# jbikker/tinybvh

Measured on NVIDIA B200. Metric: Mrays/s (primary+shadow), higher is better.
Workload: dtype f32

## Files before the change

### tinybvh_b200/csrc/common.cuh

```cuda
#pragma once
#include <cuda_runtime.h>
#include <stdint.h>
#include <stdio.h>
#include <mutex>
#include <vector>
#include <atomic>
#include "../../include/tinybvh_b200.h"

#define BVH_FAR 1e30f
#define TBVH_STACK 64
#define TBVH_STACK_DEEP 256

void tbvh_set_error( const char* fmt, ... );
extern unsigned long long g_tbvh_launches;
#define CUDA_TRY( x ) do { cudaError_t e_ = (x); if (e_ != cudaSuccess) { tbvh_set_error( "%s:%d %s -> %s", __FILE__, __LINE__, #x, cudaGetErrorString( e_ ) ); return TBVH_E_CUDA; } } while (0)
#define LAUNCHED() do { g_tbvh_launches++; cudaError_t e_ = cudaGetLastError(); if (e_ != cudaSuccess) { tbvh_set_error( "%s:%d launch -> %s", __FILE__, __LINE__, cudaGetErrorString( e_ ) ); return TBVH_E_CUDA; } } while (0)

struct HostSlot
{
	void* d_rays = 0;
	void* d_hits = 0;
	void* d_bits = 0;
	void* h_hits = 0;
	cudaEvent_t in_done = 0, run_done = 0, out_done = 0;
};
#define TBVH_SLOTS 4

struct tbvh_ctx_t
{
	int device = 0;
	int sm_count = 148;
	int numa_node = -1;
	cudaStream_t stream = 0;
	std::mutex host_mutex;
	cudaStream_t s_in = 0, s_run = 0, s_out = 0;
	cudaStream_t s_in_part[3] = { 0, 0, 0 };
	cudaEvent_t ev_part[TBVH_SLOTS][3] = {};
	cudaEvent_t ev_fork = 0;
	HostSlot slot[TBVH_SLOTS];
	size_t chunk_rays = 1u << 19;
	size_t slot_rays = 0;
	size_t slot_rec = 0;
	int host_path = 0;
	int h2d_split = 1;
	int d2h_mode = 1;
	int scatter_threads = 8;
	struct HostPool* pool = 0;
	int trace_variant = 3;
	int small_mode = 0;
	int inst_idx_bits = 32;
	int hq_small = 16;
	int hq_cluster = 16;
	int small_t = 128;
	int build_ctas = 0;
	int build_mode = 0;
	unsigned long long* d_counters = 0;
	std::atomic<uint32_t> counter_next{ 0 };
};
#define TBVH_COUNTERS 256

uint32_t tbvh_next_generation();
struct BlasLink { tbvh_bvh blas; uint32_t generation; };

struct tbvh_bvh_t
{
	tbvh_ctx ctx = 0;
	tbvh_info info = {};
	float4* d_verts = 0;
	float4* d_nodes = 0;
	uint32_t* d_prim_idx = 0;
	float4* d_trav = 0;
	uint32_t root_ref = 0, root_count = 0;
	float4* d_leaf_tris = 0;
	uint32_t leaf_tris_count = 0;
	float4* d_nodes_gpu = 0;
	float4* d_cw_nodes = 0;
	float4* d_cw_tris = 0;
	float4* d_cw_trav = 0;
	uint32_t cw_depth = 0;
	uint32_t generation = 0;
	float4* d_aabbs = 0;
	void* d_inst = 0;
	void* d_blas = 0;
	uint32_t inst_count = 0, blas_count = 0;
	uint32_t tlas_blas_layouts = 0;
	std::vector<BlasLink> links;
	bool refittable = true;
	int stats = 0;
	unsigned long long* d_stats = 0;
};


__device__ __forceinline__ bool mt_test( const float ox, const float oy, const float oz, const float dx, const float dy, const float dz,
	const float4 v0, const float4 e1, const float4 e2, const float tmax, float& t, float& u, float& v )
{
	const float hx = __fmaf_rn( dy, e2.z, -__fmul_rn( dz, e2.y ) );
	const float hy = __fmaf_rn( dz, e2.x, -__fmul_rn( dx, e2.z ) );
	const float hz = __fmaf_rn( dx, e2.y, -__fmul_rn( dy, e2.x ) );
	const float a = __fmaf_rn( e1.z, hz, __fmaf_rn( e1.x, hx, __fmul_rn( e1.y, hy ) ) );
	if (fabsf( a ) < 0.000001f) return false;
	const float f = __fdiv_rn( 1.0f, a );
	const float sx = __fsub_rn( ox, v0.x ), sy = __fsub_rn( oy, v0.y ), sz = __fsub_rn( oz, v0.z );
	u = __fmul_rn( f, __fmaf_rn( hz, sz, __fmaf_rn( hx, sx, __fmul_rn( hy, sy ) ) ) );
	const float qx = __fmaf_rn( -e1.y, sz, __fmul_rn( e1.z, sy ) );
	const float qy = __fmaf_rn( -e1.z, sx, __fmul_rn( e1.x, sz ) );
	const float qz = __fmaf_rn( -e1.x, sy, __fmul_rn( e1.y, sx ) );
	v = __fmul_rn( f, __fmaf_rn( dz, qz, __fmaf_rn( dy, qy, __fmul_rn( dx, qx ) ) ) );
	if (u < 0 || v < 0 || __fadd_rn( u, v ) > 1) return false;
	t = __fmul_rn( f, __fmaf_rn( e2.z, qz, __fmaf_rn( e2.x, qx, __fmul_rn( e2.y, qy ) ) ) );
	return !(t < 0 || t > tmax);
}

__device__ __forceinline__ uint32_t f2key( float f ) { uint32_t u = __float_as_uint( f ); return (u & 0x80000000u) ? ~u : (u | 0x80000000u); }
__device__ __forceinline__ float key2f( uint32_t k ) { return __uint_as_float( (k & 0x80000000u) ? (k & 0x7fffffffu) : ~k ); }

int bvh2_trace_launch( tbvh_bvh b, const void* d_rays, uint32_t stride, void* d_hits, uint32_t hit_stride, uint32_t* d_bits, uint64_t n, bool anyhit, cudaStream_t s, unsigned long long* d_stats );
int cwbvh_trace_launch( tbvh_bvh b, const void* d_rays, uint32_t stride, void* d_hits, uint32_t hit_stride, uint32_t* d_bits, uint64_t n, bool anyhit, cudaStream_t s, unsigned long long* d_stats );
int cw_make_trav( tbvh_bvh b, cudaStream_t s, int known_depth = -1 );
unsigned long long* ctx_next_counter( tbvh_ctx c );
int build_sah_launch( tbvh_bvh b, float c_trav, float c_int, int flavour );
int build_hq_launch( tbvh_bvh b, float c_trav, float c_int );
int refit_launch( tbvh_bvh b, cudaStream_t s );
int tlas_trace_launch( tbvh_bvh b, int layout, const void* d_rays, uint32_t stride, uint32_t* d_bits, uint64_t n, bool anyhit, cudaStream_t s );
struct TlasInst { float inv[16]; uint32_t blasIdx, mask, pad0, pad1; };
struct BlasRef { const float4* trav; const float4* tris; uint32_t root_ref, root_count, pad0, pad1; const float4* cw_nodes; const float4* cw_tris; };
int make_leaf_tris( tbvh_bvh b, cudaStream_t s );
int bvh_gpu_to_bvh( tbvh_bvh b, uint32_t used_nodes_gpu, cudaStream_t s );
int bvh_to_bvh_gpu( tbvh_bvh b, cudaStream_t s );
int bvh_to_cwbvh( tbvh_bvh b, cudaStream_t s );
int exclusive_scan( const uint32_t* in, uint32_t* out, uint32_t* tile_sum, uint32_t n, cudaStream_t s );
```

### tinybvh_b200/csrc/cw_walk.cuh

```cuda
#pragma once
#include "common.cuh"
#include <cuda_fp16.h>

#define CW_STACK 128
#define CW_NODE_F4 10
#ifndef CW_PLANES_BF16
#define CW_PLANES_BF16 0
#endif

__device__ __forceinline__ float2 widen( const uint32_t h2 )
{
#if CW_PLANES_BF16
	return make_float2( __uint_as_float( h2 * 65536u ), __uint_as_float( h2 & 0xffff0000u ) );
#else
	return __half22float2( *(const __half2*)&h2 );
#endif
}

__device__ __forceinline__ uint32_t pair_hits( const uint32_t wnx, const uint32_t wny, const uint32_t wnz, const uint32_t wfx, const uint32_t wfy, const uint32_t wfz,
	const uint32_t bits_a, const uint32_t bits_b, const float2 ax, const float2 ay, const float2 az, const float2 bx, const float2 by, const float2 bz, const float t )
{
	const float2 tnx = __ffma2_rn( widen( wnx ), ax, bx ), tny = __ffma2_rn( widen( wny ), ay, by ), tnz = __ffma2_rn( widen( wnz ), az, bz );
	const float2 tfx = __ffma2_rn( widen( wfx ), ax, bx ), tfy = __ffma2_rn( widen( wfy ), ay, by ), tfz = __ffma2_rn( widen( wfz ), az, bz );
	const float in_a = fmaxf( fmaxf( fmaxf( tnx.x, tny.x ), tnz.x ), 0.0f ), out_a = fminf( fminf( fminf( tfx.x, tfy.x ), tfz.x ), t );
	const float in_b = fmaxf( fmaxf( fmaxf( tnx.y, tny.y ), tnz.y ), 0.0f ), out_b = fminf( fminf( fminf( tfx.y, tfy.y ), tfz.y ), t );
	return (in_a <= out_a ? bits_a : 0u) | (in_b <= out_b ? bits_b : 0u);
}

__device__ __forceinline__ uint32_t slots_to_order( const uint32_t w, const uint32_t o )
{
	uint32_t top = w >> 24;
	if (o & 1u) top = ((top & 0x55u) << 1) | ((top >> 1) & 0x55u);
	if (o & 2u) top = ((top & 0x33u) << 2) | ((top >> 2) & 0x33u);
	if (o & 4u) top = ((top & 0x0fu) << 4) | (top >> 4);
	return top << 24;
}

template <int OCT> __device__ __forceinline__ uint32_t node_hits( const float4* __restrict__ np, const uint32_t pairs, const bool negx, const bool negy, const bool negz, const uint32_t o,
	const float ax1, const float ay1, const float az1, const float bx1, const float by1, const float bz1, const float t )
{
	const bool nx = OCT < 0 ? negx : (OCT & 4) != 0, ny = OCT < 0 ? negy : (OCT & 2) != 0, nz = OCT < 0 ? negz : (OCT & 1) != 0;
	const float2 ax = make_float2( ax1, ax1 ), ay = make_float2( ay1, ay1 ), az = make_float2( az1, az1 );
	const float2 bx = make_float2( bx1, bx1 ), by = make_float2( by1, by1 ), bz = make_float2( bz1, bz1 );
	(void)pairs;
	float4 A[4], B[4];
	#pragma unroll
	for (int j = 0; j < 4; j++) A[j] = __ldg( np + 2 + 2 * j ), B[j] = __ldg( np + 3 + 2 * j );
	uint32_t got = 0;
	#pragma unroll
	for (int j = 0; j < 4; j++)
	{
		const uint32_t lx = __float_as_uint( A[j].x ), ly = __float_as_uint( A[j].y ), lz = __float_as_uint( A[j].z );
		const uint32_t hx = __float_as_uint( A[j].w ), hy = __float_as_uint( B[j].x ), hz = __float_as_uint( B[j].y );
		got |= pair_hits( nx ? hx : lx, ny ? hy : ly, nz ? hz : lz, nx ? lx : hx, ny ? ly : hy, nz ? lz : hz,
			__float_as_uint( B[j].z ), __float_as_uint( B[j].w ), ax, ay, az, bx, by, bz, t );
	}
	return slots_to_order( got, OCT < 0 ? o : (uint32_t)(7 - OCT) ) | (got & 0x00ffffffu);
}
```

### tinybvh_b200/csrc/multi.cu

```cuda
#include "common.cuh"
#include <sched.h>
#include <sys/mman.h>
#include <string.h>
#include <thread>
#include <string>
#include <vector>
#include <new>

struct tbvh_group_t
{
	std::vector<tbvh_ctx> ctx;
	std::vector<tbvh_bvh> replica;
	std::vector<char> owned;
	std::vector<std::pair<void*, size_t>> host_blocks;
};

#define ARG_CHECK( c, msg ) do { if (!(c)) { tbvh_set_error( "%s: %s", __func__, msg ); return TBVH_E_ARG; } } while (0)
#define TRY( x ) do { int r_ = (x); if (r_ != TBVH_OK) return r_; } while (0)

static void release_replicas( tbvh_group g )
{
	for (size_t i = 0; i < g->replica.size(); i++) if (g->replica[i] && g->owned[i]) tbvh_bvh_destroy( g->replica[i] );
	g->replica.clear(), g->owned.clear();
}

static int peer_clone( void** dst, int dst_dev, const void* src, int src_dev, size_t bytes, cudaStream_t s )
{
	*dst = 0;
	if (!src || bytes == 0) return TBVH_OK;
	CUDA_TRY( cudaMalloc( dst, bytes ) );
	CUDA_TRY( cudaMemcpyPeerAsync( *dst, dst_dev, src, src_dev, bytes, s ) );
	return TBVH_OK;
}

template <class F> static int per_device( tbvh_group g, F fn )
{
	const size_t parts = g->ctx.size();
	std::vector<int> rc( parts, TBVH_OK );
	std::vector<std::string> msg( parts );
	std::vector<std::thread> th;
	for (size_t p = 0; p < parts; p++) th.emplace_back( [&, p]()
	{
		tbvh_bind_thread_to_device( g->ctx[p]->device );
		rc[p] = fn( (uint32_t)p );
		if (rc[p] != TBVH_OK) msg[p] = tbvh_last_error();
	} );
	for (auto& t : th) t.join();
	for (size_t p = 0; p < parts; p++) if (rc[p] != TBVH_OK) { tbvh_set_error( "device %d: %s", g->ctx[p]->device, msg[p].c_str() ); return rc[p]; }
	return TBVH_OK;
}

extern "C" {

void tbvh_shard_range( uint64_t n, uint32_t part, uint32_t parts, uint64_t* first, uint64_t* count )
{
	const uint64_t units = (n + 31) / 32;
	const uint64_t lo = units * part / parts, hi = units * (part + 1) / parts;
	const uint64_t a = lo * 32 < n ? lo * 32 : n, e = hi * 32 < n ? hi * 32 : n;
	if (first) *first = a;
	if (count) *count = e - a;
}

int tbvh_group_create( const int* devices, int count, tbvh_group* out )
{
	ARG_CHECK( out, "out == NULL" );
	int have = 0;
	CUDA_TRY( cudaGetDeviceCount( &have ) );
	if (count <= 0) count = have, devices = 0;
	ARG_CHECK( count >= 1 && count <= 64, "device count out of range" );
	for (int i = 0; i < count; i++) ARG_CHECK( (devices ? devices[i] : i) >= 0 && (devices ? devices[i] : i) < have, "no such device" );
	tbvh_group g = new (std::nothrow) tbvh_group_t();
	ARG_CHECK( g, "out of host memory" );
	for (int i = 0; i < count; i++)
	{
		const int dev = devices ? devices[i] : i;
		tbvh_ctx c = 0;
		const int rc = tbvh_ctx_create( dev, &c );
		if (rc != TBVH_OK) { for (tbvh_ctx x : g->ctx) tbvh_ctx_destroy( x ); delete g; return rc; }
		g->ctx.push_back( c );
	}
	for (int i = 0; i < count; i++) for (int j = 0; j < count; j++) if (i != j)
	{
		int can = 0;
		cudaDeviceCanAccessPeer( &can, g->ctx[i]->device, g->ctx[j]->device );
		if (can) { cudaSetDevice( g->ctx[i]->device ); if (cudaDeviceEnablePeerAccess( g->ctx[j]->device, 0 ) != cudaSuccess) cudaGetLastError(); }
	}
	*out = g;
	return TBVH_OK;
}

int tbvh_group_destroy( tbvh_group g )
{
	if (!g) return TBVH_OK;
	release_replicas( g );
	for (auto& b : g->host_blocks) { cudaHostUnregister( b.first ); munmap( b.first, b.second ); }
	for (tbvh_ctx c : g->ctx) tbvh_ctx_destroy( c );
	delete g;
	return TBVH_OK;
}

int tbvh_group_size( tbvh_group g ) { return g ? (int)g->ctx.size() : 0; }
tbvh_ctx tbvh_group_ctx( tbvh_group g, int i ) { return g && i >= 0 && i < (int)g->ctx.size() ? g->ctx[i] : 0; }
tbvh_bvh tbvh_group_replica( tbvh_group g, int i ) { return g && i >= 0 && i < (int)g->replica.size() ? g->replica[i] : 0; }

int tbvh_group_replicate( tbvh_group g, tbvh_bvh src, double* ms_out )
{
	ARG_CHECK( g && src, "NULL argument" );
	if (src->d_inst) { tbvh_set_error( "tbvh_group_replicate: a TLAS points into its BLAS handles and cannot be replicated by itself" ); return TBVH_E_UNSUPPORTED; }
	if (!(src->info.layouts & (1u << TBVH_LAYOUT_BVH)) && !src->d_cw_trav) { tbvh_set_error( "tbvh_group_replicate: the source holds no tree" ); return TBVH_E_STATE; }
	release_replicas( g );
	const int sdev = src->ctx->device;
	CUDA_TRY( cudaSetDevice( sdev ) );
	CUDA_TRY( cudaStreamSynchronize( src->ctx->stream ) );
	cudaEvent_t e0 = 0, e1 = 0;
	CUDA_TRY( cudaEventCreate( &e0 ) );
	CUDA_TRY( cudaEventCreate( &e1 ) );
	CUDA_TRY( cudaEventRecord( e0, src->ctx->stream ) );
	int rc = TBVH_OK;
	for (size_t i = 0; i < g->ctx.size() && rc == TBVH_OK; i++)
	{
		tbvh_ctx c = g->ctx[i];
		if (c == src->ctx) { g->replica.push_back( src ), g->owned.push_back( 0 ); continue; }
		tbvh_bvh r = 0;
		rc = tbvh_bvh_create( c, &r );
		if (rc != TBVH_OK) break;
		g->replica.push_back( r ), g->owned.push_back( 1 );
		auto body = [&]() -> int
		{
			CUDA_TRY( cudaSetDevice( c->device ) );
			cudaStream_t s = c->stream;
			r->info = src->info, r->root_ref = src->root_ref, r->root_count = src->root_count, r->refittable = src->refittable, r->cw_depth = src->cw_depth;
			const size_t nodes_b = (size_t)(src->info.used_nodes < 2 ? 2 : src->info.used_nodes) * 32;
			TRY( peer_clone( (void**)&r->d_verts, c->device, src->d_verts, sdev, (size_t)src->info.prim_count * 48, s ) );
			TRY( peer_clone( (void**)&r->d_prim_idx, c->device, src->d_prim_idx, sdev, (size_t)src->info.idx_count * 4, s ) );
			if (src->d_nodes) TRY( peer_clone( (void**)&r->d_nodes, c->device, src->d_nodes, sdev, nodes_b, s ) );
			if (src->d_trav == src->d_nodes) r->d_trav = r->d_nodes;
			else if (src->d_trav) TRY( peer_clone( (void**)&r->d_trav, c->device, src->d_trav, sdev, (size_t)src->info.used_nodes_gpu * 64, s ) );
			if (src->d_leaf_tris) { TRY( peer_clone( (void**)&r->d_leaf_tris, c->device, src->d_leaf_tris, sdev, (size_t)src->leaf_tris_count * 48, s ) ); r->leaf_tris_count = src->leaf_tris_count; }
			if (src->d_nodes_gpu) TRY( peer_clone( (void**)&r->d_nodes_gpu, c->device, src->d_nodes_gpu, sdev, (size_t)src->info.used_nodes_gpu * 64, s ) );
			if (src->d_cw_nodes) TRY( peer_clone( (void**)&r->d_cw_nodes, c->device, src->d_cw_nodes, sdev, (size_t)src->info.used_blocks * 16, s ) );
			if (src->d_cw_tris) TRY( peer_clone( (void**)&r->d_cw_tris, c->device, src->d_cw_tris, sdev, (size_t)src->info.cwbvh_tri_count * 48, s ) );
			if (src->d_cw_trav) TRY( peer_clone( (void**)&r->d_cw_trav, c->device, src->d_cw_trav, sdev, (size_t)(src->info.used_blocks / 5) * 160, s ) );
			return TBVH_OK;
		};
		rc = body();
	}
	for (tbvh_ctx c : g->ctx) { cudaSetDevice( c->device ); cudaStreamSynchronize( c->stream ); }
	cudaSetDevice( sdev );
	cudaEventRecord( e1, src->ctx->stream );
	cudaEventSynchronize( e1 );
	float ms = 0;
	cudaEventElapsedTime( &ms, e0, e1 );
	if (ms_out) *ms_out = ms;
	cudaEventDestroy( e0 ), cudaEventDestroy( e1 );
	if (rc != TBVH_OK) release_replicas( g );
	return rc;
}

int tbvh_group_intersect( tbvh_group g, int layout, void* rays, uint32_t stride, uint64_t n )
{
	ARG_CHECK( g && rays && stride >= 64, "bad arguments" );
	if (g->replica.size() != g->ctx.size()) { tbvh_set_error( "tbvh_group_intersect: call tbvh_group_replicate first" ); return TBVH_E_STATE; }
	const uint32_t parts = (uint32_t)g->ctx.size();
	return per_device( g, [&]( uint32_t p ) -> int
	{
		uint64_t first, count;
		tbvh_shard_range( n, p, parts, &first, &count );
		if (count == 0) return TBVH_OK;
		return tbvh_intersect( g->replica[p], layout, (char*)rays + first * stride, stride, count );
	} );
}

int tbvh_group_occluded( tbvh_group g, int layout, const void* rays, uint32_t stride, uint64_t n, uint32_t* bits )
{
	ARG_CHECK( g && rays && bits && stride >= 64, "bad arguments" );
	if (g->replica.size() != g->ctx.size()) { tbvh_set_error( "tbvh_group_occluded: call tbvh_group_replicate first" ); return TBVH_E_STATE; }
	const uint32_t parts = (uint32_t)g->ctx.size();
	return per_device( g, [&]( uint32_t p ) -> int
	{
		uint64_t first, count;
		tbvh_shard_range( n, p, parts, &first, &count );
		if (count == 0) return TBVH_OK;
		return tbvh_occluded( g->replica[p], layout, (const char*)rays + first * stride, stride, count, bits + first / 32 );
	} );
}

int tbvh_group_host_alloc( tbvh_group g, uint32_t stride, uint64_t n, void** out )
{
	ARG_CHECK( g && out && stride > 0 && n > 0, "bad arguments" );
	const size_t bytes = ((size_t)stride * n + 4095) & ~(size_t)4095;
	void* p = mmap( 0, bytes, PROT_READ | PROT_WRITE, MAP_PRIVATE | MAP_ANONYMOUS, -1, 0 );
	if (p == MAP_FAILED) { tbvh_set_error( "tbvh_group_host_alloc: mmap( %zu ) failed", bytes ); return TBVH_E_ARG; }
	const uint32_t parts = (uint32_t)g->ctx.size();
	per_device( g, [&]( uint32_t part ) -> int
	{
		uint64_t first, count;
		tbvh_shard_range( n, part, parts, &first, &count );
		char* a = (char*)p + first * stride, * e = a + count * stride;
		if (part + 1 == parts) e = (char*)p + bytes;
		for (char* q = (char*)((uintptr_t)a & ~(uintptr_t)4095); q < e; q += 4096) *(volatile char*)q = 0;
		return TBVH_OK;
	} );
	const cudaError_t err = cudaHostRegister( p, bytes, cudaHostRegisterPortable );
	if (err != cudaSuccess) { munmap( p, bytes ); tbvh_set_error( "tbvh_group_host_alloc: cudaHostRegister -> %s", cudaGetErrorString( err ) ); return TBVH_E_CUDA; }
	g->host_blocks.push_back( { p, bytes } );
	*out = p;
	return TBVH_OK;
}

int tbvh_group_host_free( tbvh_group g, void* p )
{
	ARG_CHECK( g, "NULL group" );
	for (size_t i = 0; i < g->host_blocks.size(); i++) if (g->host_blocks[i].first == p)
	{
		cudaHostUnregister( p );
		munmap( p, g->host_blocks[i].second );
		g->host_blocks.erase( g->host_blocks.begin() + i );
		return TBVH_OK;
	}
	tbvh_set_error( "tbvh_group_host_free: not a block of this group" );
	return TBVH_E_ARG;
}

}
```

### tinybvh_b200/csrc/trace_cwbvh.cu

```cuda
#include "cw_walk.cuh"
#include <vector>

__global__ void k_cw_expand( const uint4* __restrict__ src, uint4* __restrict__ dst, uint32_t* __restrict__ parent, const uint32_t count )
{
	const uint32_t x = blockIdx.x * blockDim.x + threadIdx.x;
	if (x >= count) return;
	const uint4 n0 = src[(size_t)x * 5], n1 = src[(size_t)x * 5 + 1], n2 = src[(size_t)x * 5 + 2], n3 = src[(size_t)x * 5 + 3], n4 = src[(size_t)x * 5 + 4];
	const uint32_t row[6][2] = { { n2.x, n2.y }, { n2.z, n2.w }, { n3.x, n3.y }, { n3.z, n3.w }, { n4.x, n4.y }, { n4.z, n4.w } };
	const uint32_t meta[2] = { n1.z, n1.w };
	uint32_t word[4][8];
	#pragma unroll
	for (int j = 0; j < 4; j++) for (int k = 0; k < 8; k++) word[j][k] = 0;
	uint32_t kept = 0, inner = 0;
	#pragma unroll
	for (int i = 0; i < 8; i++)
	{
		const uint32_t m = (meta[i >> 2] >> (8 * (i & 3))) & 255u;
		if (m == 0) continue;
		const bool is_inner = (m & 0x18u) == 0x18u;
		const uint32_t bits = is_inner ? 1u << (24u + (m & 7u)) : (m >> 5) << (m & 31u);
		if (is_inner) inner++;
		const uint32_t j = kept >> 1, side = kept & 1;
		#pragma unroll
		for (int r = 0; r < 6; r++)
		{
			const uint32_t q = (row[r][i >> 2] >> (8 * (i & 3))) & 255u;
			const uint32_t h = CW_PLANES_BF16 ? __float_as_uint( (float)q ) >> 16 : (uint32_t)__half_as_ushort( __uint2half_rn( q ) );
			#pragma unroll
			for (int jj = 0; jj < 4; jj++) if (jj == (int)j) word[jj][r] |= side ? h << 16 : h;
		}
		#pragma unroll
		for (int jj = 0; jj < 4; jj++) if (jj == (int)j) word[jj][6 + side] = bits;
		kept++;
	}
	uint4* o = dst + (size_t)x * CW_NODE_F4;
	const uint32_t sx = (uint32_t)(((int)(int8_t)(n0.w & 255u) + 127) * 128) & 0xffffu, sy = (uint32_t)(((int)(int8_t)((n0.w >> 8) & 255u) + 127) * 128) & 0xffffu;
	const uint32_t sz = (uint32_t)(((int)(int8_t)((n0.w >> 16) & 255u) + 127) * 128) & 0xffffu;
	o[0] = make_uint4( n0.x, n0.y, n0.z, sx | (sy << 16) );
	o[1] = make_uint4( n1.x, n1.y, sz | ((n0.w >> 24) << 16) | (((kept + 1) >> 1) << 24), kept );
	#pragma unroll
	for (int j = 0; j < 4; j++)
	{
		o[2 + 2 * j] = make_uint4( word[j][0], word[j][1], word[j][2], word[j][3] );
		o[3 + 2 * j] = make_uint4( word[j][4], word[j][5], word[j][6], word[j][7] );
	}
	if (parent) for (uint32_t c = 0; c < inner; c++) if (n1.x + c < count) parent[n1.x + c] = x;
}

__global__ void k_cw_depth( const uint32_t* __restrict__ parent, const uint32_t count, uint32_t* __restrict__ max_depth )
{
	const uint32_t x = blockIdx.x * blockDim.x + threadIdx.x;
	if (x >= count) return;
	uint32_t d = 0, n = x;
	while (n != 0 && n < count && d < 4096) n = parent[n], d++;
	if (n != 0) return;
	atomicMax( max_depth, d );
}

int cw_make_trav( tbvh_bvh b, cudaStream_t s, int known_depth )
{
	if (b->d_cw_trav) cudaFree( b->d_cw_trav ), b->d_cw_trav = 0;
	const uint32_t count = b->info.used_blocks / 5;
	if (count == 0) { tbvh_set_error( "cw_make_trav: no CWBVH nodes" ); return TBVH_E_STATE; }
	CUDA_TRY( cudaMalloc( &b->d_cw_trav, (size_t)count * CW_NODE_F4 * 16 ) );
	if (known_depth >= 0)
	{
		k_cw_expand<<<(count + 127) / 128, 128, 0, s>>>( (const uint4*)b->d_cw_nodes, (uint4*)b->d_cw_trav, 0, count ); LAUNCHED();
		b->cw_depth = (uint32_t)known_depth;
		return TBVH_OK;
	}
	uint32_t* d_parent = 0;
	CUDA_TRY( cudaMalloc( &d_parent, ((size_t)count + 1) * 4 ) );
	uint32_t depth = 0;
	auto body = [&]() -> int
	{
		CUDA_TRY( cudaMemsetAsync( d_parent, 0xff, (size_t)count * 4, s ) );
		CUDA_TRY( cudaMemsetAsync( d_parent + count, 0, 4, s ) );
		k_cw_expand<<<(count + 127) / 128, 128, 0, s>>>( (const uint4*)b->d_cw_nodes, (uint4*)b->d_cw_trav, d_parent, count ); LAUNCHED();
		k_cw_depth<<<(count + 127) / 128, 128, 0, s>>>( d_parent, count, d_parent + count ); LAUNCHED();
		CUDA_TRY( cudaMemcpyAsync( &depth, d_parent + count, 4, cudaMemcpyDeviceToHost, s ) );
		CUDA_TRY( cudaStreamSynchronize( s ) );
		return TBVH_OK;
	};
	const int rc = body();
	cudaFree( d_parent );
	b->cw_depth = depth;
	return rc;
}


template <bool ANYHIT, bool STATS, int OCTSW>
__global__ void __launch_bounds__( 128 ) k_trace_wide( const float4* __restrict__ nodes, const float4* __restrict__ tris,
	const char* rays, const uint32_t stride, char* hits, const uint32_t hit_stride, uint32_t* __restrict__ bits, const uint64_t n,
	unsigned long long* __restrict__ stats )
{
	const uint64_t i = (uint64_t)blockIdx.x * blockDim.x + threadIdx.x;
	bool occluded = false;
	const bool valid = i < n;
	float4 ro4 = make_float4( 0, 0, 0, 0 ), rd4 = ro4, rr4 = ro4, rh4 = ro4;
	if (valid)
	{
		const float4* rp = (const float4*)(rays + i * stride);
		ro4 = rp[0], rd4 = rp[1], rr4 = rp[2], rh4 = rp[3];
	}
	const float ox = ro4.x, oy = ro4.y, oz = ro4.z, dx = rd4.x, dy = rd4.y, dz = rd4.z;
	const float rdx = rr4.x, rdy = rr4.y, rdz = rr4.z;
	const uint32_t o = 7u - ((dx < 0 ? 4u : 0u) | (dy < 0 ? 2u : 0u) | (dz < 0 ? 1u : 0u));
	const bool negx = rdx < 0, negy = rdy < 0, negz = rdz < 0;
	const uint32_t oct = (negx ? 4u : 0u) | (negy ? 2u : 0u) | (negz ? 1u : 0u);
	bool uni = false;
	if (OCTSW)
	{
		const uint32_t vm = __ballot_sync( 0xffffffffu, valid );
		const uint32_t oct0 = __shfl_sync( 0xffffffffu, oct, vm ? __ffs( vm ) - 1 : 0 );
		uni = __all_sync( 0xffffffffu, !valid || (oct == oct0 && o == 7u - oct) );
	}
	if (valid)
	{
		float t = rh4.x, hu = rh4.y, hv = rh4.z;
		uint32_t hprim = __float_as_uint( rh4.w );
		uint2 pending[CW_STACK];
		int depth = 0;
		uint32_t base = 0, word = 0x80000000u;
		unsigned long long nsteps = 0, ntris = 0, npairs = 0;
		while (true)
		{
			const uint32_t bit = 31u - __clz( word );
			const uint32_t rest = word & ~(1u << bit);
			if (rest > 0x00ffffffu) pending[depth++] = make_uint2( base, rest );
			const uint32_t slot = (bit - 24u) ^ o;
			const uint32_t nidx = base + __popc( word & ~(0xffffffffu << slot) );
			const float4* np = nodes + (size_t)nidx * CW_NODE_F4;
			const float4 h0 = __ldg( np ), h1 = __ldg( np + 1 );
			if (STATS) nsteps++;
			const uint32_t sxy = __float_as_uint( h0.w ), szm = __float_as_uint( h1.z );
			const float scx = __uint_as_float( sxy << 16 ), scy = __uint_as_float( sxy & 0xffff0000u ), scz = __uint_as_float( szm << 16 );
			const float ax1 = __fmul_rn( scx, rdx ), ay1 = __fmul_rn( scy, rdy ), az1 = __fmul_rn( scz, rdz );
			const float bx1 = __fmul_rn( -__fsub_rn( ox, h0.x ), rdx ), by1 = __fmul_rn( -__fsub_rn( oy, h0.y ), rdy ), bz1 = __fmul_rn( -__fsub_rn( oz, h0.z ), rdz );
			const uint32_t pairs = szm >> 24;
			if (STATS) npairs += pairs;
			uint32_t got;
			#define NODE_HITS( O ) got = node_hits<O>( np, pairs, negx, negy, negz, o, ax1, ay1, az1, bx1, by1, bz1, t )
			if (OCTSW && uni)
			{
				switch (oct)
				{
				case 0: NODE_HITS( 0 ); break;
				case 1: NODE_HITS( 1 ); break;
				case 2: NODE_HITS( 2 ); break;
				case 3: NODE_HITS( 3 ); break;
				case 4: NODE_HITS( 4 ); break;
				case 5: NODE_HITS( 5 ); break;
				case 6: NODE_HITS( 6 ); break;
				default: NODE_HITS( 7 ); break;
				}
			}
			else NODE_HITS( -1 );
			#undef NODE_HITS
			base = __float_as_uint( h1.x );
			word = (got & 0xff000000u) | ((szm >> 16) & 255u);
			uint32_t tmask = got & 0x00ffffffu;
			const float4* tbase = tris + __float_as_uint( h1.y );
			while (tmask)
			{
				const uint32_t k = 31u - __clz( tmask );
				tmask &= ~(1u << k);
				const float4* tp = tbase + k * 3;
				const float4 e2 = __ldg( tp ), e1 = __ldg( tp + 1 ), v0 = __ldg( tp + 2 );
				if (STATS) ntris++;
				float tt, u, v;
				if (mt_test( ox, oy, oz, dx, dy, dz, v0, e1, e2, t, tt, u, v ))
				{
					if (ANYHIT) { occluded = true; break; }
					t = tt, hu = u, hv = v, hprim = __float_as_uint( v0.w );
				}
			}
			if (ANYHIT && occluded) break;
			if (word > 0x00ffffffu) continue;
			if (depth == 0) break;
			const uint2 e = pending[--depth];
			base = e.x, word = e.y;
		}
		if (!ANYHIT)
		{
			float4* hp = (float4*)(hits + i * hit_stride);
			*hp = make_float4( t, hu, hv, __uint_as_float( hprim ) );
		}
		if (STATS) { atomicAdd( &stats[0], nsteps ); atomicAdd( &stats[1], ntris ); atomicAdd( &stats[2], npairs ); }
	}
	if (ANYHIT)
	{
		const uint32_t m = __ballot_sync( 0xffffffffu, occluded );
		if ((threadIdx.x & 31) == 0 && (i & ~31ull) < n) bits[i >> 5] = m;
	}
}

int cwbvh_trace_launch( tbvh_bvh b, const void* d_rays, uint32_t stride, void* d_hits, uint32_t hit_stride, uint32_t* d_bits,
	uint64_t n, bool anyhit, cudaStream_t s, unsigned long long* d_stats )
{
	if (!b->d_cw_trav || !b->d_cw_tris) { tbvh_set_error( "CWBVH layout not resident" ); return TBVH_E_STATE; }
	if (n == 0) return TBVH_OK;
	if (b->cw_depth + 1 > CW_STACK) { tbvh_set_error( "wide-tree depth %u exceeds the %d pending node groups a ray can hold (the reference's own limit)", b->cw_depth, CW_STACK ); return TBVH_E_LIMIT; }
	const uint32_t block = 128;
	const uint64_t grid = (n + block - 1) / block;
	if (grid > 0x7fffffffull) { tbvh_set_error( "ray batch too large for one launch" ); return TBVH_E_ARG; }
	const int sw = b->ctx->trace_variant == 0 ? 0 : 1;
	#define LAUNCH( A, S, O ) k_trace_wide<A, S, O><<<(uint32_t)grid, block, 0, s>>>( b->d_cw_trav, b->d_cw_tris, (const char*)d_rays, stride, \
		(char*)d_hits, hit_stride, d_bits, n, d_stats )
	if (anyhit) { if (d_stats) LAUNCH( true, true, 0 ); else if (sw) LAUNCH( true, false, 1 ); else LAUNCH( true, false, 0 ); }
	else { if (d_stats) LAUNCH( false, true, 0 ); else if (sw) LAUNCH( false, false, 1 ); else LAUNCH( false, false, 0 ); }
	#undef LAUNCH
	LAUNCHED();
	return TBVH_OK;
}
```

### tinybvh_b200/csrc/trace_tlas.cu

```cuda
#include "cw_walk.cuh"

#define TLAS_STACK 64

namespace
{
__device__ __forceinline__ float safercp( const float x ) { return (x > 1e-12f || x < -1e-12f) ? __fdiv_rn( 1.0f, x ) : (x >= 0 ? BVH_FAR : -BVH_FAR); }

__device__ __forceinline__ bool slab( const float4 c0, const float4 c1, const bool px, const bool py, const bool pz, const float rdx, const float rdy, const float rdz,
	const float nrox, const float nroy, const float nroz, const float tmax, float& tmin )
{
	const float tx1 = __fmaf_rn( px ? c0.x : c1.x, rdx, nrox ), tx2 = __fmaf_rn( px ? c1.x : c0.x, rdx, nrox );
	const float ty1 = __fmaf_rn( py ? c0.y : c1.y, rdy, nroy ), ty2 = __fmaf_rn( py ? c1.y : c0.y, rdy, nroy );
	const float tz1 = __fmaf_rn( pz ? c0.z : c1.z, rdz, nroz ), tz2 = __fmaf_rn( pz ? c1.z : c0.z, rdz, nroz );
	tmin = fmaxf( fmaxf( tx1, ty1 ), fmaxf( tz1, 0.0f ) );
	return fminf( fminf( tx2, ty2 ), fminf( tz2, tmax ) ) >= tmin;
}

template <bool ANYHIT> __device__ bool trace_blas( const BlasRef B, const float ox, const float oy, const float oz, const float dx, const float dy, const float dz,
	const float rdx, const float rdy, const float rdz, float& tmax, float& hu, float& hv, uint32_t& hprim, bool& hit, uint2* stack )
{
	const bool px = dx >= 0, py = dy >= 0, pz = dz >= 0;
	const float nrox = -__fmul_rn( ox, rdx ), nroy = -__fmul_rn( oy, rdy ), nroz = -__fmul_rn( oz, rdz );
	int sp = 0;
	uint32_t ref = B.root_ref, cnt = B.root_count;
	while (true)
	{
		if (cnt == 0)
		{
			const float4* p = B.trav + (size_t)ref * 2;
			const float4 a0 = __ldg( p ), a1 = __ldg( p + 1 ), b0 = __ldg( p + 2 ), b1 = __ldg( p + 3 );
			float tmina, tminb;
			const bool hita = slab( a0, a1, px, py, pz, rdx, rdy, rdz, nrox, nroy, nroz, tmax, tmina );
			const bool hitb = slab( b0, b1, px, py, pz, rdx, rdy, rdz, nrox, nroy, nroz, tmax, tminb );
			const uint32_t refa = __float_as_uint( a0.w ), cnta = __float_as_uint( a1.w ), refb = __float_as_uint( b0.w ), cntb = __float_as_uint( b1.w );
			if (hita && hitb)
			{
				const bool swp = tmina > tminb;
				ref = swp ? refb : refa, cnt = swp ? cntb : cnta;
				stack[sp++] = swp ? make_uint2( refa, cnta ) : make_uint2( refb, cntb );
				continue;
			}
			if (hita) { ref = refa, cnt = cnta; continue; }
			if (hitb) { ref = refb, cnt = cntb; continue; }
		}
		else
		{
			const float4* tp = B.tris + (size_t)ref * 3;
			for (uint32_t k = 0; k < cnt; k++, tp += 3)
			{
				const float4 v0 = __ldg( tp ), e1 = __ldg( tp + 1 ), e2 = __ldg( tp + 2 );
				float t, u, v;
				if (mt_test( ox, oy, oz, dx, dy, dz, v0, e1, e2, tmax, t, u, v ))
				{
					if (ANYHIT) return true;
					tmax = t, hu = u, hv = v, hprim = __float_as_uint( v0.w ), hit = true;
				}
			}
		}
		if (sp == 0) break;
		const uint2 e = stack[--sp];
		ref = e.x, cnt = e.y;
	}
	return false;
}

template <bool ANYHIT> __device__ bool trace_blas_cw( const float4* __restrict__ nodes, const float4* __restrict__ tris, const float ox, const float oy, const float oz,
	const float dx, const float dy, const float dz, const float rdx, const float rdy, const float rdz, float& tmax, float& hu, float& hv, uint32_t& hprim, bool& hit, uint2* pending )
{
	const uint32_t o = 7u - ((dx < 0 ? 4u : 0u) | (dy < 0 ? 2u : 0u) | (dz < 0 ? 1u : 0u));
	const bool negx = rdx < 0, negy = rdy < 0, negz = rdz < 0;
	const float t_in = tmax;
	float t = tmax, lu = 0, lv = 0;
	uint32_t lprim = 0;
	int depth = 0;
	uint32_t base = 0, word = 0x80000000u;
	while (true)
	{
		const uint32_t bit = 31u - __clz( word );
		const uint32_t rest = word & ~(1u << bit);
		if (rest > 0x00ffffffu) pending[depth++] = make_uint2( base, rest );
		const uint32_t slot = (bit - 24u) ^ o;
		const uint32_t nidx = base + __popc( word & ~(0xffffffffu << slot) );
		const float4* np = nodes + (size_t)nidx * CW_NODE_F4;
		const float4 h0 = __ldg( np ), h1 = __ldg( np + 1 );
		const uint32_t sxy = __float_as_uint( h0.w ), szm = __float_as_uint( h1.z );
		const float scx = __uint_as_float( sxy << 16 ), scy = __uint_as_float( sxy & 0xffff0000u ), scz = __uint_as_float( szm << 16 );
		const float ax1 = __fmul_rn( scx, rdx ), ay1 = __fmul_rn( scy, rdy ), az1 = __fmul_rn( scz, rdz );
		const float bx1 = __fmul_rn( -__fsub_rn( ox, h0.x ), rdx ), by1 = __fmul_rn( -__fsub_rn( oy, h0.y ), rdy ), bz1 = __fmul_rn( -__fsub_rn( oz, h0.z ), rdz );
		const uint32_t got = node_hits<-1>( np, szm >> 24, negx, negy, negz, o, ax1, ay1, az1, bx1, by1, bz1, t );
		base = __float_as_uint( h1.x );
		word = (got & 0xff000000u) | ((szm >> 16) & 255u);
		uint32_t tmask = got & 0x00ffffffu;
		const float4* tbase = tris + __float_as_uint( h1.y );
		while (tmask)
		{
			const uint32_t k = 31u - __clz( tmask );
			tmask &= ~(1u << k);
			const float4* tp = tbase + k * 3;
			const float4 e2 = __ldg( tp ), e1 = __ldg( tp + 1 ), v0 = __ldg( tp + 2 );
			float tt, u, v;
			if (mt_test( ox, oy, oz, dx, dy, dz, v0, e1, e2, t, tt, u, v ))
			{
				if (ANYHIT) { if (tt < t_in) return true; }
				else t = tt, lu = u, lv = v, lprim = __float_as_uint( v0.w );
			}
		}
		if (word > 0x00ffffffu) continue;
		if (depth == 0) break;
		const uint2 e = pending[--depth];
		base = e.x, word = e.y;
	}
	if (!ANYHIT && t < t_in) tmax = t, hu = lu, hv = lv, hprim = lprim, hit = true;
	return false;
}

template <bool ANYHIT, bool CW> __global__ void __launch_bounds__( 128 ) k_trace_tlas( const float4* __restrict__ nodes, const uint32_t* __restrict__ prim_idx,
	const TlasInst* __restrict__ inst, const BlasRef* __restrict__ blas, char* rays, const uint32_t stride, uint32_t* __restrict__ bits, const uint64_t n,
	const uint32_t root_ref, const uint32_t root_count, const uint32_t inst_shift  )
{
	const uint64_t i = (uint64_t)blockIdx.x * blockDim.x + threadIdx.x;
	bool occluded = false;
	if (i < n)
	{
		const float4* rp = (const float4*)(rays + i * stride);
		const float4 ro4 = rp[0], rd4 = rp[1], rr4 = rp[2], rh4 = rp[3];
		const float ox = ro4.x, oy = ro4.y, oz = ro4.z, dx = rd4.x, dy = rd4.y, dz = rd4.z, rdx = rr4.x, rdy = rr4.y, rdz = rr4.z;
		const uint32_t rmask = __float_as_uint( ro4.w );
		const bool px = dx >= 0, py = dy >= 0, pz = dz >= 0;
		const float nrox = -__fmul_rn( ox, rdx ), nroy = -__fmul_rn( oy, rdy ), nroz = -__fmul_rn( oz, rdz );
		float tmax = rh4.x, hu = rh4.y, hv = rh4.z;
		uint32_t hprim = __float_as_uint( rh4.w ), hinst = __float_as_uint( rr4.w );
		uint2 stack[TLAS_STACK], bstack[CW ? CW_STACK : TBVH_STACK];
		int sp = 0;
		uint32_t ref = root_ref, cnt = root_count;
		while (true)
		{
			if (cnt == 0)
			{
				const float4* p = nodes + (size_t)ref * 2;
				const float4 a0 = __ldg( p ), a1 = __ldg( p + 1 ), b0 = __ldg( p + 2 ), b1 = __ldg( p + 3 );
				float tmina, tminb;
				const bool hita = slab( a0, a1, px, py, pz, rdx, rdy, rdz, nrox, nroy, nroz, tmax, tmina );
				const bool hitb = slab( b0, b1, px, py, pz, rdx, rdy, rdz, nrox, nroy, nroz, tmax, tminb );
				const uint32_t refa = __float_as_uint( a0.w ), cnta = __float_as_uint( a1.w ), refb = __float_as_uint( b0.w ), cntb = __float_as_uint( b1.w );
				if (hita && hitb)
				{
					const bool swp = tmina > tminb;
					ref = swp ? refb : refa, cnt = swp ? cntb : cnta;
					stack[sp++] = swp ? make_uint2( refa, cnta ) : make_uint2( refb, cntb );
					continue;
				}
				if (hita) { ref = refa, cnt = cnta; continue; }
				if (hitb) { ref = refb, cnt = cntb; continue; }
			}
			else
			{
				for (uint32_t k = 0; k < cnt; k++)
				{
					const uint32_t instIdx = __ldg( prim_idx + ref + k );
					const float4* ip = (const float4*)(inst + instIdx);
					const float4 r0 = __ldg( ip ), r1 = __ldg( ip + 1 ), r2 = __ldg( ip + 2 ), r3 = __ldg( ip + 3 ), meta = __ldg( ip + 4 );
					if (!(__float_as_uint( meta.y ) & rmask)) continue;
					float tox = __fadd_rn( __fmaf_rn( r0.z, oz, __fmaf_rn( r0.x, ox, __fmul_rn( r0.y, oy ) ) ), r0.w );
					float toy = __fadd_rn( __fmaf_rn( r1.z, oz, __fmaf_rn( r1.x, ox, __fmul_rn( r1.y, oy ) ) ), r1.w );
					float toz = __fadd_rn( __fmaf_rn( r2.z, oz, __fmaf_rn( r2.x, ox, __fmul_rn( r2.y, oy ) ) ), r2.w );
					const float w = __fadd_rn( __fmaf_rn( oz, r3.z, __fmaf_rn( ox, r3.x, __fmul_rn( oy, r3.y ) ) ), r3.w );
					if (!(w == 1.0f)) { const float rw = __fdiv_rn( 1.0f, w ); tox = __fmul_rn( tox, rw ), toy = __fmul_rn( toy, rw ), toz = __fmul_rn( toz, rw ); }
					const float tdx = __fmaf_rn( r0.z, dz, __fmaf_rn( r0.x, dx, __fmul_rn( r0.y, dy ) ) );
					const float tdy = __fmaf_rn( r1.z, dz, __fmaf_rn( r1.x, dx, __fmul_rn( r1.y, dy ) ) );
					const float tdz = __fmaf_rn( r2.z, dz, __fmaf_rn( r2.x, dx, __fmul_rn( r2.y, dy ) ) );
					bool hit = false;
					const BlasRef B = blas[__float_as_uint( meta.x )];
					const bool occ = CW ? trace_blas_cw<ANYHIT>( B.cw_nodes, B.cw_tris, tox, toy, toz, tdx, tdy, tdz, safercp( tdx ), safercp( tdy ), safercp( tdz ), tmax, hu, hv, hprim, hit, bstack )
						: trace_blas<ANYHIT>( B, tox, toy, toz, tdx, tdy, tdz, safercp( tdx ), safercp( tdy ), safercp( tdz ), tmax, hu, hv, hprim, hit, bstack );
					if (occ)
					{
						occluded = true;
						break;
					}
					if (hit)
					{
						hinst = instIdx;
						if (inst_shift) hprim += instIdx << inst_shift;
					}
				}
				if (ANYHIT && occluded) break;
			}
			if (sp == 0) break;
			const uint2 e = stack[--sp];
			ref = e.x, cnt = e.y;
		}
		if (!ANYHIT)
		{
			char* rec = rays + i * stride;
			if (inst_shift == 0) *(uint32_t*)(rec + 44) = hinst;
			*(float4*)(rec + 48) = make_float4( tmax, hu, hv, __uint_as_float( hprim ) );
		}
	}
	if (ANYHIT)
	{
		const uint32_t m = __ballot_sync( 0xffffffffu, occluded );
		if ((threadIdx.x & 31) == 0 && (i & ~31ull) < n) bits[i >> 5] = m;
	}
}
}

int tlas_trace_launch( tbvh_bvh b, int layout, const void* d_rays, uint32_t stride, uint32_t* d_bits, uint64_t n, bool anyhit, cudaStream_t s )
{
	if (!b->d_inst || !b->d_blas || !b->d_nodes) { tbvh_set_error( "TLAS not resident" ); return TBVH_E_STATE; }
	const bool cw = layout == TBVH_LAYOUT_CWBVH;
	if (!cw && layout != TBVH_LAYOUT_BVH && layout != TBVH_LAYOUT_BVH_GPU) { tbvh_set_error( "unknown layout %d", layout ); return TBVH_E_ARG; }
	if (cw && !(b->tlas_blas_layouts & (1u << TBVH_LAYOUT_CWBVH)))
	{ tbvh_set_error( "TLAS: not every BLAS held its CWBVH layout when the TLAS was built (tbvh_convert the BLASses, then tbvh_build_tlas)" ); return TBVH_E_STATE; }
	if (!cw && !(b->tlas_blas_layouts & (1u << TBVH_LAYOUT_BVH)))
	{ tbvh_set_error( "TLAS: not every BLAS holds a BVH-layout tree; walk it with TBVH_LAYOUT_CWBVH" ); return TBVH_E_STATE; }
	if (n == 0) return TBVH_OK;
	const uint64_t grid = (n + 127) / 128;
	if (grid > 0x7fffffffull) { tbvh_set_error( "ray batch too large for one launch" ); return TBVH_E_ARG; }
	const int bits_opt = b->ctx->inst_idx_bits;
	const uint32_t shift = bits_opt >= 4 && bits_opt < 32 ? (uint32_t)(32 - bits_opt) : 0u;
	#define LAUNCH( A, C ) k_trace_tlas<A, C><<<(uint32_t)grid, 128, 0, s>>>( b->d_nodes, b->d_prim_idx, (const TlasInst*)b->d_inst, (const BlasRef*)b->d_blas, \
		(char*)d_rays, stride, d_bits, n, b->root_ref, b->root_count, shift )
	if (anyhit) { if (cw) LAUNCH( true, true ); else LAUNCH( true, false ); }
	else { if (cw) LAUNCH( false, true ); else LAUNCH( false, false ); }
	#undef LAUNCH
	LAUNCHED();
	return TBVH_OK;
}
```

Measured before the change: 3616.

## Store CWBVH child planes as fp32 SoA and load with 256-bit vector loads

The traversal node layout changes from 10 float4 with packed fp16 quantized planes interleaved per child pair to 16 float4 holding fp32 planes in structure-of-arrays chunks of 8 children, read with ld.global.nc.v8 (32-byte) loads. The half-to-float widening goes away and the ray direction's octant picks whole plane chunks, so the near/far swizzle per child pair is no longer needed. The cost is a 60% larger node footprint, more memory and cache traffic per visited node, and reliance on 256-bit load support.

```diff
diff --git a/tinybvh_b200/csrc/common.cuh b/tinybvh_b200/csrc/common.cuh
--- a/tinybvh_b200/csrc/common.cuh
+++ b/tinybvh_b200/csrc/common.cuh
@@ -10,6 +10,7 @@
 #define BVH_FAR 1e30f
 #define TBVH_STACK 64
 #define TBVH_STACK_DEEP 256
+#define CW_NODE_F4 16
 
 void tbvh_set_error( const char* fmt, ... );
 extern unsigned long long g_tbvh_launches;
diff --git a/tinybvh_b200/csrc/cw_walk.cuh b/tinybvh_b200/csrc/cw_walk.cuh
--- a/tinybvh_b200/csrc/cw_walk.cuh
+++ b/tinybvh_b200/csrc/cw_walk.cuh
@@ -1,30 +1,23 @@
 #pragma once
 #include "common.cuh"
-#include <cuda_fp16.h>
 
 #define CW_STACK 128
-#define CW_NODE_F4 10
-#ifndef CW_PLANES_BF16
-#define CW_PLANES_BF16 0
-#endif
+#define CW_HITS 1
+#define CW_LO 2
+#define CW_HI 5
 
-__device__ __forceinline__ float2 widen( const uint32_t h2 )
+__device__ __forceinline__ void ldg8( const float4* p, float4& a, float4& b )
 {
-#if CW_PLANES_BF16
-	return make_float2( __uint_as_float( h2 * 65536u ), __uint_as_float( h2 & 0xffff0000u ) );
-#else
-	return __half22float2( *(const __half2*)&h2 );
-#endif
+	asm( "ld.global.nc.v8.f32 {%0, %1, %2, %3, %4, %5, %6, %7}, [%8];"
+		: "=f"( a.x ), "=f"( a.y ), "=f"( a.z ), "=f"( a.w ), "=f"( b.x ), "=f"( b.y ), "=f"( b.z ), "=f"( b.w ) : "l"( p ) );
 }
 
-__device__ __forceinline__ uint32_t pair_hits( const uint32_t wnx, const uint32_t wny, const uint32_t wnz, const uint32_t wfx, const uint32_t wfy, const uint32_t wfz,
-	const uint32_t bits_a, const uint32_t bits_b, const float2 ax, const float2 ay, const float2 az, const float2 bx, const float2 by, const float2 bz, const float t )
+__device__ __forceinline__ void plane_t( const float4* np, const int chunk, const float2 a, const float2 b, float2 r[4] )
 {
-	const float2 tnx = __ffma2_rn( widen( wnx ), ax, bx ), tny = __ffma2_rn( widen( wny ), ay, by ), tnz = __ffma2_rn( widen( wnz ), az, bz );
-	const float2 tfx = __ffma2_rn( widen( wfx ), ax, bx ), tfy = __ffma2_rn( widen( wfy ), ay, by ), tfz = __ffma2_rn( widen( wfz ), az, bz );
-	const float in_a = fmaxf( fmaxf( fmaxf( tnx.x, tny.x ), tnz.x ), 0.0f ), out_a = fminf( fminf( fminf( tfx.x, tfy.x ), tfz.x ), t );
-	const float in_b = fmaxf( fmaxf( fmaxf( tnx.y, tny.y ), tnz.y ), 0.0f ), out_b = fminf( fminf( fminf( tfx.y, tfy.y ), tfz.y ), t );
-	return (in_a <= out_a ? bits_a : 0u) | (in_b <= out_b ? bits_b : 0u);
+	float4 c0, c1;
+	ldg8( np + 2 * chunk, c0, c1 );
+	r[0] = __ffma2_rn( make_float2( c0.x, c0.y ), a, b ), r[1] = __ffma2_rn( make_float2( c0.z, c0.w ), a, b );
+	r[2] = __ffma2_rn( make_float2( c1.x, c1.y ), a, b ), r[3] = __ffma2_rn( make_float2( c1.z, c1.w ), a, b );
 }
 
 __device__ __forceinline__ uint32_t slots_to_order( const uint32_t w, const uint32_t o )
@@ -36,24 +29,32 @@
 	return top << 24;
 }
 
-template <int OCT> __device__ __forceinline__ uint32_t node_hits( const float4* __restrict__ np, const uint32_t pairs, const bool negx, const bool negy, const bool negz, const uint32_t o,
+template <int OCT> __device__ __forceinline__ uint32_t node_hits( const float4* __restrict__ np, const bool negx, const bool negy, const bool negz, const uint32_t o,
 	const float ax1, const float ay1, const float az1, const float bx1, const float by1, const float bz1, const float t )
 {
 	const bool nx = OCT < 0 ? negx : (OCT & 4) != 0, ny = OCT < 0 ? negy : (OCT & 2) != 0, nz = OCT < 0 ? negz : (OCT & 1) != 0;
 	const float2 ax = make_float2( ax1, ax1 ), ay = make_float2( ay1, ay1 ), az = make_float2( az1, az1 );
 	const float2 bx = make_float2( bx1, bx1 ), by = make_float2( by1, by1 ), bz = make_float2( bz1, bz1 );
-	(void)pairs;
-	float4 A[4], B[4];
+	float2 in[4], out[4], tp[4];
+	plane_t( np, nx ? CW_HI : CW_LO, ax, bx, in );
+	plane_t( np, ny ? CW_HI + 1 : CW_LO + 1, ay, by, tp );
 	#pragma unroll
-	for (int j = 0; j < 4; j++) A[j] = __ldg( np + 2 + 2 * j ), B[j] = __ldg( np + 3 + 2 * j );
+	for (int j = 0; j < 4; j++) in[j] = make_float2( fmaxf( in[j].x, tp[j].x ), fmaxf( in[j].y, tp[j].y ) );
+	plane_t( np, nz ? CW_HI + 2 : CW_LO + 2, az, bz, tp );
+	#pragma unroll
+	for (int j = 0; j < 4; j++) in[j] = make_float2( fmaxf( fmaxf( in[j].x, tp[j].x ), 0.0f ), fmaxf( fmaxf( in[j].y, tp[j].y ), 0.0f ) );
+	plane_t( np, nx ? CW_LO : CW_HI, ax, bx, out );
+	plane_t( np, ny ? CW_LO + 1 : CW_HI + 1, ay, by, tp );
+	#pragma unroll
+	for (int j = 0; j < 4; j++) out[j] = make_float2( fminf( out[j].x, tp[j].x ), fminf( out[j].y, tp[j].y ) );
+	plane_t( np, nz ? CW_LO + 2 : CW_HI + 2, az, bz, tp );
+	#pragma unroll
+	for (int j = 0; j < 4; j++) out[j] = make_float2( fminf( fminf( out[j].x, tp[j].x ), t ), fminf( fminf( out[j].y, tp[j].y ), t ) );
+	float4 w0, w1;
+	ldg8( np + 2 * CW_HITS, w0, w1 );
+	const float w[8] = { w0.x, w0.y, w0.z, w0.w, w1.x, w1.y, w1.z, w1.w };
 	uint32_t got = 0;
 	#pragma unroll
-	for (int j = 0; j < 4; j++)
-	{
-		const uint32_t lx = __float_as_uint( A[j].x ), ly = __float_as_uint( A[j].y ), lz = __float_as_uint( A[j].z );
-		const uint32_t hx = __float_as_uint( A[j].w ), hy = __float_as_uint( B[j].x ), hz = __float_as_uint( B[j].y );
-		got |= pair_hits( nx ? hx : lx, ny ? hy : ly, nz ? hz : lz, nx ? lx : hx, ny ? ly : hy, nz ? lz : hz,
-			__float_as_uint( B[j].z ), __float_as_uint( B[j].w ), ax, ay, az, bx, by, bz, t );
-	}
+	for (int j = 0; j < 4; j++) got |= (in[j].x <= out[j].x ? __float_as_uint( w[2 * j] ) : 0u) | (in[j].y <= out[j].y ? __float_as_uint( w[2 * j + 1] ) : 0u);
 	return slots_to_order( got, OCT < 0 ? o : (uint32_t)(7 - OCT) ) | (got & 0x00ffffffu);
 }
diff --git a/tinybvh_b200/csrc/multi.cu b/tinybvh_b200/csrc/multi.cu
--- a/tinybvh_b200/csrc/multi.cu
+++ b/tinybvh_b200/csrc/multi.cu
@@ -140,7 +140,7 @@
 			if (src->d_nodes_gpu) TRY( peer_clone( (void**)&r->d_nodes_gpu, c->device, src->d_nodes_gpu, sdev, (size_t)src->info.used_nodes_gpu * 64, s ) );
 			if (src->d_cw_nodes) TRY( peer_clone( (void**)&r->d_cw_nodes, c->device, src->d_cw_nodes, sdev, (size_t)src->info.used_blocks * 16, s ) );
 			if (src->d_cw_tris) TRY( peer_clone( (void**)&r->d_cw_tris, c->device, src->d_cw_tris, sdev, (size_t)src->info.cwbvh_tri_count * 48, s ) );
-			if (src->d_cw_trav) TRY( peer_clone( (void**)&r->d_cw_trav, c->device, src->d_cw_trav, sdev, (size_t)(src->info.used_blocks / 5) * 160, s ) );
+			if (src->d_cw_trav) TRY( peer_clone( (void**)&r->d_cw_trav, c->device, src->d_cw_trav, sdev, (size_t)(src->info.used_blocks / 5) * CW_NODE_F4 * 16, s ) );
 			return TBVH_OK;
 		};
 		rc = body();
diff --git a/tinybvh_b200/csrc/trace_cwbvh.cu b/tinybvh_b200/csrc/trace_cwbvh.cu
--- a/tinybvh_b200/csrc/trace_cwbvh.cu
+++ b/tinybvh_b200/csrc/trace_cwbvh.cu
@@ -8,9 +8,9 @@
 	const uint4 n0 = src[(size_t)x * 5], n1 = src[(size_t)x * 5 + 1], n2 = src[(size_t)x * 5 + 2], n3 = src[(size_t)x * 5 + 3], n4 = src[(size_t)x * 5 + 4];
 	const uint32_t row[6][2] = { { n2.x, n2.y }, { n2.z, n2.w }, { n3.x, n3.y }, { n3.z, n3.w }, { n4.x, n4.y }, { n4.z, n4.w } };
 	const uint32_t meta[2] = { n1.z, n1.w };
-	uint32_t word[4][8];
+	uint32_t word[7][8];
 	#pragma unroll
-	for (int j = 0; j < 4; j++) for (int k = 0; k < 8; k++) word[j][k] = 0;
+	for (int c = 0; c < 7; c++) for (int k = 0; k < 8; k++) word[c][k] = 0;
 	uint32_t kept = 0, inner = 0;
 	#pragma unroll
 	for (int i = 0; i < 8; i++)
@@ -20,17 +20,13 @@
 		const bool is_inner = (m & 0x18u) == 0x18u;
 		const uint32_t bits = is_inner ? 1u << (24u + (m & 7u)) : (m >> 5) << (m & 31u);
 		if (is_inner) inner++;
-		const uint32_t j = kept >> 1, side = kept & 1;
 		#pragma unroll
-		for (int r = 0; r < 6; r++)
+		for (int k = 0; k < 8; k++) if (k == (int)kept)
 		{
-			const uint32_t q = (row[r][i >> 2] >> (8 * (i & 3))) & 255u;
-			const uint32_t h = CW_PLANES_BF16 ? __float_as_uint( (float)q ) >> 16 : (uint32_t)__half_as_ushort( __uint2half_rn( q ) );
+			word[0][k] = bits;
 			#pragma unroll
-			for (int jj = 0; jj < 4; jj++) if (jj == (int)j) word[jj][r] |= side ? h << 16 : h;
+			for (int r = 0; r < 6; r++) word[1 + r][k] = __float_as_uint( (float)((row[r][i >> 2] >> (8 * (i & 3))) & 255u) );
 		}
-		#pragma unroll
-		for (int jj = 0; jj < 4; jj++) if (jj == (int)j) word[jj][6 + side] = bits;
 		kept++;
 	}
 	uint4* o = dst + (size_t)x * CW_NODE_F4;
@@ -39,10 +35,10 @@
 	o[0] = make_uint4( n0.x, n0.y, n0.z, sx | (sy << 16) );
 	o[1] = make_uint4( n1.x, n1.y, sz | ((n0.w >> 24) << 16) | (((kept + 1) >> 1) << 24), kept );
 	#pragma unroll
-	for (int j = 0; j < 4; j++)
-	{
-		o[2 + 2 * j] = make_uint4( word[j][0], word[j][1], word[j][2], word[j][3] );
-		o[3 + 2 * j] = make_uint4( word[j][4], word[j][5], word[j][6], word[j][7] );
+	for (int c = 0; c < 7; c++)
+	{
+		o[2 + 2 * c] = make_uint4( word[c][0], word[c][1], word[c][2], word[c][3] );
+		o[3 + 2 * c] = make_uint4( word[c][4], word[c][5], word[c][6], word[c][7] );
 	}
 	if (parent) for (uint32_t c = 0; c < inner; c++) if (n1.x + c < count) parent[n1.x + c] = x;
 }
@@ -131,7 +127,8 @@
 			const uint32_t slot = (bit - 24u) ^ o;
 			const uint32_t nidx = base + __popc( word & ~(0xffffffffu << slot) );
 			const float4* np = nodes + (size_t)nidx * CW_NODE_F4;
-			const float4 h0 = __ldg( np ), h1 = __ldg( np + 1 );
+			float4 h0, h1;
+			ldg8( np, h0, h1 );
 			if (STATS) nsteps++;
 			const uint32_t sxy = __float_as_uint( h0.w ), szm = __float_as_uint( h1.z );
 			const float scx = __uint_as_float( sxy << 16 ), scy = __uint_as_float( sxy & 0xffff0000u ), scz = __uint_as_float( szm << 16 );
@@ -140,7 +137,7 @@
 			const uint32_t pairs = szm >> 24;
 			if (STATS) npairs += pairs;
 			uint32_t got;
-			#define NODE_HITS( O ) got = node_hits<O>( np, pairs, negx, negy, negz, o, ax1, ay1, az1, bx1, by1, bz1, t )
+			#define NODE_HITS( O ) got = node_hits<O>( np, negx, negy, negz, o, ax1, ay1, az1, bx1, by1, bz1, t )
 			if (OCTSW && uni)
 			{
 				switch (oct)
diff --git a/tinybvh_b200/csrc/trace_tlas.cu b/tinybvh_b200/csrc/trace_tlas.cu
--- a/tinybvh_b200/csrc/trace_tlas.cu
+++ b/tinybvh_b200/csrc/trace_tlas.cu
@@ -82,12 +82,13 @@
 		const uint32_t slot = (bit - 24u) ^ o;
 		const uint32_t nidx = base + __popc( word & ~(0xffffffffu << slot) );
 		const float4* np = nodes + (size_t)nidx * CW_NODE_F4;
-		const float4 h0 = __ldg( np ), h1 = __ldg( np + 1 );
+		float4 h0, h1;
+		ldg8( np, h0, h1 );
 		const uint32_t sxy = __float_as_uint( h0.w ), szm = __float_as_uint( h1.z );
 		const float scx = __uint_as_float( sxy << 16 ), scy = __uint_as_float( sxy & 0xffff0000u ), scz = __uint_as_float( szm << 16 );
 		const float ax1 = __fmul_rn( scx, rdx ), ay1 = __fmul_rn( scy, rdy ), az1 = __fmul_rn( scz, rdz );
 		const float bx1 = __fmul_rn( -__fsub_rn( ox, h0.x ), rdx ), by1 = __fmul_rn( -__fsub_rn( oy, h0.y ), rdy ), bz1 = __fmul_rn( -__fsub_rn( oz, h0.z ), rdz );
-		const uint32_t got = node_hits<-1>( np, szm >> 24, negx, negy, negz, o, ax1, ay1, az1, bx1, by1, bz1, t );
+		const uint32_t got = node_hits<-1>( np, negx, negy, negz, o, ax1, ay1, az1, bx1, by1, bz1, t );
 		base = __float_as_uint( h1.x );
 		word = (got & 0xff000000u) | ((szm >> 16) & 255u);
 		uint32_t tmask = got & 0x00ffffffu;
```

After: 3069 (median of 6 runs). -15.1%, worse.
